# fluent/chunkio

Measured on AMD Instinct MI355X. Metric: device-resident CRC32 GB/s over N×400KB chunks; % HBM-read roofline, higher is better.
Workload: dtype u8

## Files before the change

chunkio_amd/_lib.py:

```python
import ctypes
import os
import sys

HERE = os.path.dirname(os.path.abspath(__file__))
LIB_PATH = os.environ.get("CIO_AMD_LIB") or os.path.join(HERE, "lib", "libchunkio_amd.so")

EXPORTS = (
    "crc_update",
    "cio_gpu_init", "cio_gpu_last_error", "cio_gpu_version",
    "cio_crc32_shift", "cio_crc32_combine",
    "cio_crc32_plan_create", "cio_crc32_plan_destroy", "cio_crc32_plan_exec",
    "cio_crc32_plan_exec_events", "cio_crc32_plan_bytes", "cio_crc32_plan_kernel", "cio_crc32_plan_aligned", "cio_crc32_plan_workgroups", "cio_crc32_ring_create", "cio_crc32_ring_exec",
    "cio_crc32_ring_join", "cio_crc32_ring_destroy", "cio_crc32_batch_dev", "cio_crc32_batch_host",
    "cio_crc32_devplan_create", "cio_crc32_devplan_destroy", "cio_crc32_devplan_exec", "cio_crc32_devplan_workgroups",
    "cio_crc32_batch_host_multi", "cio_crc32_split_host_multi", "cio_crc32_batch_fd_multi", "cio_gpu_device_count", "cio_gpu_set_device", "cio_gpu_get_device", "cio_gpu_numa_node",
    "cio_gpu_pci_bus_id", "cio_gpu_plan_cache_stats",
    "cio_crc32_host_register", "cio_crc32_host_unregister", "cio_gpu_pipe_last_timing",
    "cio_crc32_cpu_max", "cio_crc32_set_cpu_max", "cio_crc32_split_route", "cio_crc32_set_split_route", "cio_crc32_split_rates", "cio_crc32_split_forget", "cio_crc32_host_threads", "cio_crc32_set_host_threads",
    "cio_crc32_route_reset",
    "cio_crc32_batch_cpu", "cio_crc32_batch_fd_cpu",
    "cio_gpu_fill_synthetic", "cio_sha1_batch_dev", "cio_sha1_batch_dev_async",
    "cio_sha1_state_init", "cio_sha1_update_batch_dev", "cio_sha1_final_batch_dev", "cio_gpu_read_stream", "cio_gpu_read_stream_grid",
    "cio_gpu_event_create", "cio_gpu_event_destroy", "cio_gpu_event_record",
    "cio_gpu_event_elapsed_ms", "cio_gpu_stream_sync",
    "cio_sha1_init", "cio_sha1_update", "cio_sha1_final", "cio_sha1_hash", "cio_sha1_to_hex",
    "cioa_SHA1_Init", "cioa_SHA1_Update", "cioa_SHA1_Final",
    "cio_file_verify_batch", "cio_file_verify_batch_multi", "cio_verify_paths", "cio_verify_paths_multi",
    "cio_file_verify_batch_dev",
    "cio_dev_writer_create", "cio_dev_writer_destroy", "cio_file_init_batch_dev", "cio_file_write_batch_dev",
    "cio_file_seal_batch_dev",
    "cio_dev_writer_create_ex", "cio_dev_writer_move_segments", "cio_file_write_metadata_batch_dev",
    "cio_file_write_at_batch_dev",
    "cio_file_write_records_batch_dev",
    "cio_file_write_records_ungrouped_batch_dev",
    "cio_file_grow_batch_dev", "cio_file_grow_records_batch_dev",
    "cio_file_read_batch_dev", "cio_file_read_packed_batch_dev", "cio_meta_cmp_batch_dev",
    "cio_file_sync_batch", "cio_file_sync_batch_multi", "cio_file_sync_batch_begin", "cio_file_sync_batch_end",
    "cioa_create", "cioa_destroy", "cioa_set_max_chunks_up", "cioa_set_realloc_size_hint",
    "cioa_enable_file_trimming", "cioa_disable_file_trimming", "cioa_get_flags", "cioa_set_devices",
    "cioa_last_chunk_error", "cioa_total_chunks", "cioa_total_chunks_up",
    "cioa_stream_create", "cioa_stream_get", "cioa_stream_size_chunks_up", "cioa_stream_chunks", "cioa_scan_stream", "cioa_scan_streams", "cioa_scan_dump",
    "cioa_chunk_open", "cioa_chunk_close", "cioa_chunk_delete", "cioa_chunk_write", "cioa_chunk_write_at",
    "cioa_chunk_sync", "cioa_chunk_sync_batch", "cioa_chunk_sync_batch_begin", "cioa_chunk_sync_batch_end",
    "cioa_chunk_get_content", "cioa_chunk_get_content_copy",
    "cioa_chunk_get_content_size", "cioa_chunk_get_content_end_pos", "cioa_chunk_is_file",
    "cioa_chunk_close_stream", "cioa_chunk_get_real_size", "cioa_chunk_hash", "cioa_chunk_lock",
    "cioa_chunk_unlock", "cioa_chunk_is_locked", "cioa_chunk_tx_begin", "cioa_chunk_tx_commit",
    "cioa_chunk_tx_rollback", "cioa_chunk_is_up", "cioa_chunk_up", "cioa_chunk_up_force",
    "cioa_chunk_up_batch", "cioa_chunk_up_force_batch", "cioa_chunk_down",
    "cioa_chunk_name", "cioa_chunk_map", "cioa_error_get", "cioa_chunk_crc_cur", "cioa_chunk_set_crc_cur",
    "cioa_meta_write", "cioa_meta_read", "cioa_meta_cmp", "cioa_meta_size", "cioa_bench_perf_write",
)

_lib = None
_hip_runtime = None

c_u64_p = ctypes.POINTER(ctypes.c_uint64)
c_u32_p = ctypes.POINTER(ctypes.c_uint32)


def _bind(lib):
    V, P = ctypes.c_void_p, ctypes.POINTER
    sig = {
        "crc_update": (ctypes.c_uint64, [ctypes.c_uint64, V, ctypes.c_size_t]),
        "cio_gpu_init": (ctypes.c_int, []),
        "cio_gpu_last_error": (ctypes.c_char_p, []),
        "cio_gpu_version": (ctypes.c_char_p, []),
        "cio_crc32_shift": (ctypes.c_uint32, [ctypes.c_uint32, ctypes.c_uint64]),
        "cio_crc32_combine": (ctypes.c_uint32, [ctypes.c_uint32, ctypes.c_uint32, ctypes.c_uint64]),
        "cio_crc32_plan_create": (ctypes.c_int, [P(V), c_u64_p, c_u64_p, ctypes.c_size_t]),
        "cio_crc32_plan_destroy": (None, [V]),
        "cio_crc32_plan_exec": (ctypes.c_int, [V, V, V, V, V]),
        "cio_crc32_plan_exec_events": (ctypes.c_int, [V, V, V, V, V, V, V]),
        "cio_crc32_plan_bytes": (ctypes.c_uint64, [V]),
        "cio_crc32_plan_kernel": (ctypes.c_char_p, [V]),
        "cio_crc32_plan_workgroups": (ctypes.c_uint32, [V]),
        "cio_crc32_plan_aligned": (ctypes.c_int, [V]),
        "cio_crc32_ring_create": (ctypes.c_int, [ctypes.POINTER(V), ctypes.POINTER(ctypes.c_uint64),
                                                 ctypes.POINTER(ctypes.c_uint64), ctypes.c_size_t, ctypes.c_int]),
        "cio_crc32_ring_exec": (ctypes.c_int, [V, V, V, V, V]),
        "cio_crc32_ring_join": (ctypes.c_int, [V, V]),
        "cio_crc32_ring_destroy": (None, [V]),
        "cio_crc32_batch_dev": (ctypes.c_int, [V, c_u64_p, c_u64_p, V, V, ctypes.c_size_t, V]),
        "cio_crc32_devplan_create": (ctypes.c_int, [P(V), ctypes.c_size_t]),
        "cio_crc32_devplan_destroy": (None, [V]),
        "cio_crc32_devplan_exec": (ctypes.c_int, [V, V, ctypes.c_uint64, V, V, ctypes.c_size_t, V, V, V, V]),
        "cio_crc32_devplan_workgroups": (ctypes.c_uint32, [V]),
        "cio_file_verify_batch_dev": (ctypes.c_int, [V, V, ctypes.c_uint64, V, V, ctypes.c_size_t, ctypes.c_int,
                                                     V, V, V, V, V, V]),
        "cio_dev_writer_create": (ctypes.c_int, [P(V), ctypes.c_size_t]),
        "cio_dev_writer_destroy": (None, [V]),
        "cio_file_init_batch_dev": (ctypes.c_int, [V, V, ctypes.c_uint64, V, V, ctypes.c_size_t, V, ctypes.c_uint64,
                                                   V, V, ctypes.c_int, V, V, V]),
        "cio_file_write_batch_dev": (ctypes.c_int, [V, V, ctypes.c_uint64, V, V, ctypes.c_size_t, V, ctypes.c_uint64,
                                                    V, V, ctypes.c_int, V, V, V]),
        "cio_file_seal_batch_dev": (ctypes.c_int, [V, V, ctypes.c_uint64, V, V, ctypes.c_size_t, ctypes.c_int,
                                                   V, V, V]),
        "cio_dev_writer_create_ex": (ctypes.c_int, [P(V), ctypes.c_size_t, ctypes.c_int]),
        "cio_dev_writer_move_segments": (ctypes.c_uint32, [V]),
        "cio_file_write_metadata_batch_dev": (ctypes.c_int, [V, V, ctypes.c_uint64, V, V, ctypes.c_size_t, V,
                                                             ctypes.c_uint64, V, V, ctypes.c_int, V, V, V]),
        "cio_file_write_at_batch_dev": (ctypes.c_int, [V, V, ctypes.c_uint64, V, V, ctypes.c_size_t, V, V,
                                                       ctypes.c_uint64, V, V, ctypes.c_int, V, V, V]),
        "cio_file_write_records_batch_dev": (ctypes.c_int, [V, V, ctypes.c_uint64, V, V, ctypes.c_size_t, V,
                                                            ctypes.c_uint64, V, V, V, ctypes.c_size_t, ctypes.c_int,
                                                            V, V, V, V]),
        "cio_file_write_records_ungrouped_batch_dev": (ctypes.c_int, [V, V, ctypes.c_uint64, V, V, ctypes.c_size_t,
                                                                      V, ctypes.c_uint64, V, V, V, ctypes.c_size_t,
                                                                      ctypes.c_int, V, V, V, V, V]),
        "cio_file_grow_batch_dev": (ctypes.c_int, [V, V, ctypes.c_uint64, V, V, ctypes.c_size_t, V, V,
                                                   ctypes.c_uint64, ctypes.c_uint64, ctypes.c_uint64, ctypes.c_int,
                                                   V, V, V, V, V]),
        "cio_file_grow_records_batch_dev": (ctypes.c_int, [V, V, ctypes.c_uint64, V, V, ctypes.c_size_t, V, V,
                                                           ctypes.c_size_t, V, ctypes.c_uint64, ctypes.c_uint64,
                                                           ctypes.c_uint64, ctypes.c_int, V, V, V, V, V]),
        "cio_file_read_batch_dev": (ctypes.c_int, [V, V, ctypes.c_uint64, V, V, ctypes.c_size_t, ctypes.c_int, V,
                                                   V, ctypes.c_uint64, V, V, ctypes.c_int, V, V, V]),
        "cio_file_read_packed_batch_dev": (ctypes.c_int, [V, V, ctypes.c_uint64, V, V, ctypes.c_size_t, ctypes.c_int,
                                                          V, V, ctypes.c_uint64, ctypes.c_uint64, ctypes.c_int, V, V,
                                                          V, V, V]),
        "cio_meta_cmp_batch_dev": (ctypes.c_int, [V, ctypes.c_uint64, V, V, ctypes.c_size_t, V, ctypes.c_uint64, V,
                                                  V, V, V, V]),
        "cio_crc32_batch_host": (ctypes.c_int, [P(V), P(ctypes.c_size_t), c_u32_p, c_u32_p,
                                                ctypes.c_size_t]),
        "cio_crc32_batch_host_multi": (ctypes.c_int, [P(V), P(ctypes.c_size_t), c_u32_p, c_u32_p,
                                                      ctypes.c_size_t, P(ctypes.c_int), ctypes.c_int]),
        "cio_crc32_split_host_multi": (ctypes.c_int, [V, ctypes.c_size_t, ctypes.c_uint32, c_u32_p,
                                                      P(ctypes.c_int), ctypes.c_int]),
        "cio_gpu_device_count": (ctypes.c_int, []),
        "cio_gpu_set_device": (ctypes.c_int, [ctypes.c_int]),
        "cio_gpu_get_device": (ctypes.c_int, []),
        "cio_gpu_numa_node": (ctypes.c_int, [ctypes.c_int]),
        "cio_gpu_pci_bus_id": (ctypes.c_int, [ctypes.c_int, ctypes.c_char_p, ctypes.c_int]),
        "cio_gpu_plan_cache_stats": (ctypes.c_int, [ctypes.POINTER(ctypes.c_uint64), ctypes.c_int]),
        "cio_crc32_host_register": (ctypes.c_int, [V, ctypes.c_size_t]),
        "cio_crc32_host_unregister": (ctypes.c_int, [V]),
        "cio_gpu_pipe_last_timing": (ctypes.c_int, [P(ctypes.c_double), ctypes.c_int]),
        "cio_crc32_cpu_max": (ctypes.c_size_t, []),
        "cio_crc32_set_cpu_max": (None, [ctypes.c_size_t]),
        "cio_crc32_split_route": (ctypes.c_int, []),
        "cio_crc32_set_split_route": (None, [ctypes.c_int]),
        "cio_crc32_split_rates": (None, [ctypes.POINTER(ctypes.c_double), ctypes.c_int]),
        "cio_crc32_split_forget": (None, []),
        "cio_crc32_host_threads": (ctypes.c_int, []),
        "cio_crc32_set_host_threads": (None, [ctypes.c_int]),
        "cio_crc32_route_reset": (None, []),
        "cio_crc32_batch_cpu": (ctypes.c_int, [P(V), P(ctypes.c_size_t), c_u32_p, c_u32_p, ctypes.c_size_t,
                                               ctypes.c_int]),
        "cio_crc32_batch_fd_cpu": (ctypes.c_int, [P(ctypes.c_int), c_u64_p, P(ctypes.c_size_t), c_u32_p, c_u32_p,
                                                  ctypes.c_size_t, ctypes.c_int]),
        "cio_gpu_fill_synthetic": (ctypes.c_int, [V, c_u64_p, c_u64_p, c_u64_p, ctypes.c_size_t,
                                                  ctypes.c_uint64, V]),
        "cio_sha1_batch_dev": (ctypes.c_int, [V, c_u64_p, c_u64_p, V, ctypes.c_size_t, V]),
        "cio_sha1_batch_dev_async": (ctypes.c_int, [V, V, V, V, ctypes.c_size_t, V]),
        "cio_sha1_state_init": (None, [V, ctypes.c_size_t]),
        "cio_sha1_update_batch_dev": (ctypes.c_int, [V, V, V, V, ctypes.c_size_t, V]),
        "cio_sha1_final_batch_dev": (ctypes.c_int, [V, V, ctypes.c_size_t, V]),
        "cio_sha1_init": (None, [V]),
        "cio_sha1_update": (None, [V, V, ctypes.c_ulong]),
        "cio_sha1_final": (None, [V, V]),
# ... 98 lines not shown
```

chunkio_amd/crc32.py:

```python
import ctypes

import numpy as np

from . import _lib

CRC_INIT = 0xFFFFFFFF


def crc_init():
    return CRC_INIT


def crc_finalize(crc):
    return (crc ^ 0xFFFFFFFF) & 0xFFFFFFFF


def _as_bytes(data):
    if isinstance(data, np.ndarray):
        return np.ascontiguousarray(data).view(np.uint8)
    return np.frombuffer(memoryview(data).cast("B"), dtype=np.uint8)


def crc_update(crc, data):
    buf = _as_bytes(data)
    ptr = buf.ctypes.data if buf.size else None
    return int(_lib.lib().crc_update(crc & 0xFFFFFFFFFFFFFFFF, ptr, buf.size))


def crc32(data, seed=CRC_INIT):
    return crc_finalize(crc_update(seed, data))


def crc32_shift(raw_state, nbytes):
    return int(_lib.lib().cio_crc32_shift(raw_state & 0xFFFFFFFF, nbytes))


def crc32_combine(raw_a, raw0_b, len_b):
    return int(_lib.lib().cio_crc32_combine(raw_a & 0xFFFFFFFF, raw0_b & 0xFFFFFFFF, len_b))


def _u64_array(values):
    arr = np.ascontiguousarray(np.asarray(values, dtype=np.uint64))
    return arr, arr.ctypes.data_as(_lib.c_u64_p)


def _ptr(t):
    return None if t is None else ctypes.c_void_p(t.data_ptr())


def _stream_ptr(stream):
    if stream is None:
        import torch
        stream = torch.cuda.current_stream()
    return ctypes.c_void_p(int(stream.cuda_stream))


class Crc32Plan:

    def __init__(self, offs, lens):
        self._offs, po = _u64_array(offs)
        self._lens, pl = _u64_array(lens)
        if self._offs.shape != self._lens.shape:
            raise ValueError("offs and lens must have the same length")
        self.n = int(self._offs.size)
        handle = ctypes.c_void_p()
        _lib.check(_lib.lib().cio_crc32_plan_create(ctypes.byref(handle), po, pl, self.n),
                   "cio_crc32_plan_create")
        self._handle = handle

    @property
    def bytes(self):
        return int(_lib.lib().cio_crc32_plan_bytes(self._handle))

    @property
    def workgroups(self):
        return int(_lib.lib().cio_crc32_plan_workgroups(self._handle))

    def kernel_name(self):
        return _lib.lib().cio_crc32_plan_kernel(self._handle).decode()

    @property
    def aligned(self):
        return bool(_lib.lib().cio_crc32_plan_aligned(self._handle))

    def exec(self, base, out, seeds=None, stream=None):
        _lib.check(_lib.lib().cio_crc32_plan_exec(self._handle, _ptr(base), _ptr(seeds), _ptr(out),
                                                  _stream_ptr(stream)),
                   "cio_crc32_plan_exec")

    def exec_events(self, base, out, ev_start, ev_stop, seeds=None, stream=None):
        _lib.check(_lib.lib().cio_crc32_plan_exec_events(self._handle, _ptr(base), _ptr(seeds),
                                                         _ptr(out), _stream_ptr(stream),
                                                         ev_start, ev_stop),
                   "cio_crc32_plan_exec_events")

    def close(self):
        if getattr(self, "_handle", None):
            _lib.lib().cio_crc32_plan_destroy(self._handle)
            self._handle = None

    def __del__(self):
        try:
            self.close()
        except Exception:
            pass

    def __enter__(self):
        return self

    def __exit__(self, *exc):
        self.close()


class Crc32Ring:

    def __init__(self, offs, lens, depth=2):
        self._offs, po = _u64_array(offs)
        self._lens, pl = _u64_array(lens)
        if self._offs.shape != self._lens.shape:
            raise ValueError("offs and lens must have the same length")
        self.n = int(self._offs.size)
        handle = ctypes.c_void_p()
        _lib.check(_lib.lib().cio_crc32_ring_create(ctypes.byref(handle), po, pl, self.n, int(depth)),
                   "cio_crc32_ring_create")
        self._handle = handle

    def exec(self, base, out, seeds=None, stream=None):
        _lib.check(_lib.lib().cio_crc32_ring_exec(self._handle, _ptr(base), _ptr(seeds), _ptr(out),
                                                  _stream_ptr(stream)),
                   "cio_crc32_ring_exec")

    def join(self, stream=None):
        _lib.check(_lib.lib().cio_crc32_ring_join(self._handle, _stream_ptr(stream)), "cio_crc32_ring_join")

    def close(self):
        if getattr(self, "_handle", None):
            _lib.lib().cio_crc32_ring_destroy(self._handle)
            self._handle = None

    def __del__(self):
        try:
            self.close()
        except Exception:
            pass

    def __enter__(self):
        return self

    def __exit__(self, *exc):
        self.close()


DEVPLAN_E_BOUNDS, DEVPLAN_E_CHUNK_TOO_LARGE, DEVPLAN_E_BATCH_TOO_LARGE = 1, 2, 4


class Crc32DevPlan:

    def __init__(self, max_chunks):
        self.max_chunks = int(max_chunks)
        handle = ctypes.c_void_p()
        _lib.check(_lib.lib().cio_crc32_devplan_create(ctypes.byref(handle), self.max_chunks),
                   "cio_crc32_devplan_create")
        self._handle = handle
        import torch
        self._status = torch.zeros(1, dtype=torch.int32, device=torch.device("cuda", torch.cuda.current_device()))

# ... 304 lines not shown
```

chunkio_amd/csrc/cio_plan.h:

```cpp
#ifndef CIOA_PLAN_H
#define CIOA_PLAN_H

#include <stddef.h>
#include <stdint.h>
#include <vector>

#include "cio_diag.h"
#include "crc32_host.h"
#include "chunkio_amd/cio_crc32_gpu.h"

namespace cioa {

constexpr int kWave = 64;
constexpr int kGran = 16;
constexpr int kSub = 4;
constexpr int kRow = kWave * kGran;
constexpr int kStep = kSub * kRow;
constexpr int kThreads = 1024;
constexpr uint32_t kWavesPerWg = kThreads / kWave;
constexpr uint32_t kWfFold = 1u, kWfPublish = 2u;
constexpr int kX8Count = 2 * kStep;
constexpr uint32_t kSliceBytes = 131072;
constexpr uint32_t kShiftBytes = 32768;
constexpr uint32_t kShiftOff = kSliceBytes;
constexpr uint32_t kLdsBytes = kSliceBytes + kShiftBytes;
constexpr int kStampWords = 16;

struct ChunkDesc {
    uint64_t a;
    uint64_t vlen;
    uint64_t g;
    uint32_t nsteps;
    uint32_t h;
    uint32_t npieces;
    uint32_t w0, w1;
    uint32_t pad;
};
static_assert(sizeof(ChunkDesc) == 48, "desc layout");

struct WaveStart {
    ChunkDesc d;
    uint32_t c;
    uint32_t pad[3];
};
static_assert(sizeof(WaveStart) == 64, "wave start layout");

struct DeviceState {
    bool ready = false;
    int cus = 0;
    uint32_t *slice = nullptr;
    uint32_t *shift = nullptr;
    uint32_t *x8 = nullptr;
    uint32_t *xinv8 = nullptr;
};

struct PlanHost {
    std::vector<ChunkDesc> desc;
    std::vector<WaveStart> ws;
    std::vector<uint32_t> tiny;
    std::vector<uint32_t> pfac;
    std::vector<uint32_t> afac;
    uint64_t S = 0, bytes = 0;
};

void plan_init(cio_crc32_plan *p, DeviceState *st, size_t n);
const char *plan_build(PlanHost &ph, const uint64_t *offs, const uint64_t *lens, size_t n, uint32_t W);
const char *plan_choose(cio_crc32_plan *p, PlanHost &ph, const uint64_t *offs, const uint64_t *lens, size_t n);

constexpr int kDevHdrS = 0, kDevHdrNtiny = 1, kDevHdrBytes = 2, kDevHdrStatus = 3, kDevHdrWords = 4;
constexpr uint32_t kPlanBlock = 1024;

struct PlanBlockSum {
    uint64_t steps, bytes;
    uint32_t ntiny, err;
};

}

struct cio_crc32_plan {
    uint32_t n = 0;
    uint64_t S = 0;
    uint32_t W = 0;
    uint32_t grid = 0;
    uint32_t ntiny = 0;
    int prio = 1;
    uint64_t ustride = 0, ua0 = 0, uvlen = 0;
    uint32_t unsteps = 0, uh = 0;
    bool small = false;
    bool ahead = false;
    bool l64 = false;
    bool l64_small = false;
    bool aligned = false;
    uint32_t aq = 0, alg2p = 0;
    uint32_t *afac = nullptr;
    unsigned long long *stamps = nullptr;
    uint64_t bytes = 0;
    cioa::ChunkDesc *desc = nullptr;
    cioa::WaveStart *wstart = nullptr;
    uint32_t *tiny = nullptr;
    unsigned long long *partials = nullptr;
    uint32_t *counters = nullptr;
    uint32_t *pfac = nullptr;
    cioa::DeviceState *st = nullptr;
};

#endif
```

chunkio_amd/csrc/crc32_gpu.hip:

```cpp

#include <hip/hip_runtime.h>
#include <stdint.h>
#include <algorithm>
#include <type_traits>

#include "cio_gpu_internal.h"
#include "crc_wave.h"

using namespace cioa;

namespace {


constexpr uint32_t cx_multmodp(uint32_t a, uint32_t b)
{
    uint32_t p = 0;
    for (int i = 31; i >= 0; --i) {
        if ((a >> i) & 1u) {
            p ^= b;
        }
        b = (b & 1u) ? (b >> 1) ^ CIOA_POLY : (b >> 1);
    }
    return p;
}
// ... 1119 lines not shown
        if (L64) {
            const uint4 k1 = head_fix(make_uint4(~0u, ~0u, ~0u, ~0u), g0 + 1u, uh, 0u);
            const uint4 x1 = head_fix(make_uint4(0u, 0u, 0u, 0u), g0 + 1u, uh, 0xffffffffu);
            hk1[0] = k1.x; hk1[1] = k1.y; hk1[2] = k1.z; hk1[3] = k1.w;
            hs1[0] = x1.x; hs1[1] = x1.y; hs1[2] = x1.z; hs1[3] = x1.w;
        }
    }
    __syncthreads();

    auto chunk = [&](SmallRegs &cur, uint32_t c) {
        uint64_t a;
        uint32_t vlen, h;
        bool live;
        geom(c < c1 ? c : max(c1, 1u) - 1u, a, vlen, h, live);
        live = live && c < c1;
        uint32_t st = 0;
        const uint32_t seed = SEEDS ? cur.seed : 0xffffffffu;
        if (live) {
            StepRegs r;
#pragma unroll
            for (int q = 0; q < kSub; ++q) {
                r.q[q] = cur.q[q];
            }
            if (L64) {
                transpose64(r);
            }
            if (UNI && !SEEDS) {
                r.q[0] = make_uint4((r.q[0].x & hk[0]) ^ hs[0], (r.q[0].y & hk[1]) ^ hs[1],
                                    (r.q[0].z & hk[2]) ^ hs[2], (r.q[0].w & hk[3]) ^ hs[3]);
                if (L64) {
                    r.q[1] = make_uint4((r.q[1].x & hk1[0]) ^ hs1[0], (r.q[1].y & hk1[1]) ^ hs1[1],
                                        (r.q[1].z & hk1[2]) ^ hs1[2], (r.q[1].w & hk1[3]) ^ hs1[3]);
                }
            } else if (L64) {
                r.q[0] = head_fix(r.q[0], 4u * lane, h, seed);
                r.q[1] = head_fix(r.q[1], 4u * lane + 1u, h, seed);
            } else {
                r.q[0] = head_fix(r.q[0], lane, h, seed);
            }
            if (vlen < (uint32_t) kStep) {
#pragma unroll
                for (int q = 0; q < kSub; ++q) {
                    r.q[q] = mask_tail(r.q[q], L64 ? 64u * lane + 16u * (uint32_t) q : lbyte + (uint32_t) q * kRow,
                                       vlen);
                }
            }
            st = block16(lds, lb_lo, lb_hi, 0u, r.q[0]);
#pragma unroll
            for (int q = 1; q < kSub; ++q) {
                st = L64 ? block16(lds, lb_lo, lb_hi, st, r.q[q])
                         : shift_block16(lds, lb_lo, lb_hi, lrep, st, r.q[q]);
            }
        }
        uint32_t inv = inv_u;
        if (!UNI) {
            asm volatile("v_mov_b32 %0, %1" : "=v"(inv) : "v"(cur.inv));
        }
        issue(cur, c + 1);
        if (live) {
            uint32_t x = col[0] & (0u - (st & 1u));
#pragma unroll
            for (int j = 1; j < 32; ++j) {
                x = xor_and(x, 0u - ((st >> j) & 1u), col[j]);
            }
            uint32_t crc = wave_xor(x);
            if (vlen != (uint32_t) kStep) {
                asm volatile("" : "+v"(inv));
                crc = multmodp(inv, crc);
            }
            if (lane == 0) {
                out[c] = crc;
            }
        }
    };
    const uint32_t slot_group = __builtin_amdgcn_readfirstlane((tid >> 6) >> 2);
    for (uint32_t c = c0; c < c1; ++c) {
        rotate_prio(slot_group, c - c0);
        chunk(cur, c);
    }
    __builtin_amdgcn_s_setprio(0);
    tiny_chunks(lds, lb_lo, base, desc, tiny, seeds, out, nullptr, ntiny, wave, lane, W);
}


}

extern "C" {

int cioa_debug_stamps(const cio_crc32_plan *p, unsigned long long *host, size_t cap)
{
    if (!p || !p->stamps) {
        return 0;
    }
    const size_t n = std::min(cap, (size_t) p->W * kStampWords);
    if (hipMemcpy(host, p->stamps, n * sizeof(unsigned long long), hipMemcpyDeviceToHost) != hipSuccess) {
        return 0;
    }
    return (int) p->W;
}

int cioa_debug_plan_exec_cid(const cio_crc32_plan *p, const void *dev_base, const uint32_t *dev_seeds,
                             uint32_t *dev_out, const uint32_t *dev_cid, void *stream)
{
    return plan_exec_impl(p, dev_base, dev_seeds, dev_out, dev_cid, reinterpret_cast<hipStream_t>(stream));
}

}

using StreamKernel = decltype(&crc32_stream_kernel<false, 1, false>);

static StreamKernel select_kernel(int prio, bool stamps, bool uniform, bool ahead, bool l64)
{
    if (ahead) {
        if (l64) {
            if (stamps) {
                return crc32_stream_kernel<true, 1, true, true, true>;
            }
            return prio ? crc32_stream_kernel<false, 1, true, true, true>
                        : crc32_stream_kernel<false, 0, true, true, true>;
        }
        return prio ? crc32_stream_kernel<false, 1, true, true> : crc32_stream_kernel<false, 0, true, true>;
    }
    if (l64 && !stamps) {
        return prio ? crc32_stream_kernel<false, 1, false, false, true>
                    : crc32_stream_kernel<false, 0, false, false, true>;
    }
    switch ((prio ? 4 : 0) + (stamps ? 2 : 0) + (uniform ? 1 : 0)) {
    case 0: return crc32_stream_kernel<false, 0, false>;
    case 1: return crc32_stream_kernel<false, 0, true>;
    case 2: return crc32_stream_kernel<true, 0, false>;
    case 3: return crc32_stream_kernel<true, 0, true>;
    case 4: return crc32_stream_kernel<false, 1, false>;
    case 5: return crc32_stream_kernel<false, 1, true>;
    case 6: return crc32_stream_kernel<true, 1, false>;
    default: return crc32_stream_kernel<true, 1, true>;
    }
}


int cioa::plan_exec_impl(const cio_crc32_plan *p, const void *dev_base, const uint32_t *dev_seeds,
                         uint32_t *dev_out, const uint32_t *cid, hipStream_t s,
                         hipEvent_t ev0, hipEvent_t ev1)
{
    if (!p) {
        return fail("cio_crc32_plan_exec: null plan");
    }
    if (p->n == 0) {
        return CIO_OK;
    }
    if (!dev_base || !dev_out) {
        return fail("cio_crc32_plan_exec: null buffer");
    }
    const DeviceState *st = p->st;
    if (ev0) {
        HIP_TRY(hipEventRecord(ev0, s), "hipEventRecord");
    }
    if (p->small && !cid) {
        auto sk = p->l64_small ? (p->unsteps ? (dev_seeds ? crc32_small_kernel<true, true, true>
                                                    : crc32_small_kernel<true, false, true>)
                                       : (dev_seeds ? crc32_small_kernel<false, true, true>
                                                    : crc32_small_kernel<false, false, true>))
                         : (p->unsteps ? (dev_seeds ? crc32_small_kernel<true, true> : crc32_small_kernel<true, false>)
                                       : (dev_seeds ? crc32_small_kernel<false, true>
                                                    : crc32_small_kernel<false, false>));
        hipLaunchKernelGGL(sk, dim3(p->grid), dim3(kThreads), 0, s,
                           reinterpret_cast<const uint8_t *>(dev_base), p->ustride, p->ua0, p->uvlen, p->uh,
                           p->W, p->n, p->ntiny, st->x8, p->desc, p->tiny, dev_seeds, dev_out, st->xinv8);
        HIP_TRY(hipGetLastError(), "crc32_small_kernel launch");
        if (ev1) {
            HIP_TRY(hipEventRecord(ev1, s), "hipEventRecord");
        }
        return CIO_OK;
    }
    if (p->aligned) {
        auto ak = p->stamps ? crc32_aligned_kernel<true> : crc32_aligned_kernel<false>;
        hipLaunchKernelGGL(ak, dim3(p->grid), dim3(kThreads), 0, s, reinterpret_cast<const uint8_t *>(dev_base),
                           p->ustride, p->ua0, p->aq, p->alg2p, p->afac, dev_seeds, dev_out, cid, p->stamps);
        HIP_TRY(hipGetLastError(), "crc32_aligned_kernel launch");
        if (ev1) {
            HIP_TRY(hipEventRecord(ev1, s), "hipEventRecord");
        }
        return CIO_OK;
    }
    auto kern = select_kernel(p->prio, p->stamps != nullptr, p->unsteps != 0, p->ahead && (!p->stamps || p->l64),
                              p->l64);
    hipLaunchKernelGGL(kern, dim3(p->grid), dim3(kThreads), 0, s,
                       reinterpret_cast<const uint8_t *>(dev_base), p->S, p->ustride, p->ua0, p->uvlen,
                       p->W, p->unsteps, p->uh, p->n, p->desc, p->wstart, p->tiny,
                       dev_seeds, dev_out, cid, p->partials, p->counters, st->slice, st->shift,
                       st->x8, p->pfac, p->ntiny, p->stamps);
    HIP_TRY(hipGetLastError(), "crc32_stream_kernel launch");
    if (ev1) {
        HIP_TRY(hipEventRecord(ev1, s), "hipEventRecord");
    }
    return CIO_OK;
}

int cioa::devplan_crc_launch(const cio_crc32_plan *p, const unsigned long long *hdr, const void *dev_base,
                             const uint32_t *dev_seeds, uint32_t *dev_out, size_t n, hipStream_t s)
{
    const DeviceState *st = p->st;
    StreamKernel kern = p->l64 ? (p->prio ? crc32_stream_kernel<false, 1, false, false, true, true>
                                          : crc32_stream_kernel<false, 0, false, false, true, true>)
                               : (p->prio ? crc32_stream_kernel<false, 1, false, false, false, true>
                                          : crc32_stream_kernel<false, 0, false, false, false, true>);
    hipLaunchKernelGGL(kern, dim3(p->grid), dim3(kThreads), 0, s,
                       reinterpret_cast<const uint8_t *>(dev_base), (uint64_t) 0, (uint64_t) 0, (uint64_t) 0,
                       (uint64_t) 0, p->W, 0u, 0u, (uint32_t) n, p->desc, p->wstart, p->tiny,
                       dev_seeds, dev_out, (const uint32_t *) nullptr, p->partials, p->counters, st->slice,
                       st->shift, st->x8, p->pfac, 0u, const_cast<unsigned long long *>(hdr));
    HIP_TRY(hipGetLastError(), "crc32_stream_kernel (device-planned) launch");
    return CIO_OK;
}
```

chunkio_amd/csrc/crc_plan.cpp:

```cpp

#include <stdint.h>
#include <stdlib.h>
#include <string.h>
#include <algorithm>
#include <vector>

#include "cio_plan.h"

namespace cioa {

void plan_init(cio_crc32_plan *p, DeviceState *st, size_t n)
{
    p->st = st;
    p->n = (uint32_t) n;
    if (const char *r = cioa_diag_getenv("CIO_GPU_PRIO")) {
        const int v = atoi(r);
        p->prio = (v == 0) ? 0 : 1;
    }
    p->l64 = true;
    p->l64_small = false;
    if (const char *r = cioa_diag_getenv("CIO_GPU_L64")) {
        p->l64 = p->l64_small = atoi(r) != 0;
    }
    p->grid = (uint32_t) st->cus;
// ... 145 lines not shown
    p->ustride = stride;
    p->ua0 = ph.desc[0].a;
    p->uvlen = ph.desc[0].vlen;
    p->uh = ph.desc[0].h;
    p->unsteps = ph.desc[0].nsteps;
}

}

const char *plan_choose(cio_crc32_plan *p, PlanHost &ph, const uint64_t *offs, const uint64_t *lens, size_t n)
{
    if (const char *err = plan_build(ph, offs, lens, n, p->W)) {
        return err;
    }
    plan_uniform(p, offs, lens, n, ph);
    auto small_batch = [&ph, n] { return ph.S > 0 && ph.S == (uint64_t) n - ph.tiny.size(); };
    bool oversub = false;
    if (!cioa_diag_getenv("CIO_GPU_GRID") && ph.S >= 1024ull * p->W && 4ull * p->W <= 65536 &&
        !small_batch()) {
        PlanHost ph4;
        if (plan_build(ph4, offs, lens, n, 4 * p->W) == nullptr) {
            p->grid *= 4;
            p->W *= 4;
            oversub = true;
            ph = std::move(ph4);
        }
    }
    {
        const char *r = cioa_diag_getenv("CIO_GPU_ANTICAMP");
        const bool on = !(r && atoi(r) == 0);
        const char *mx = cioa_diag_getenv("CIO_GPU_ANTICAMP_MAX");
        const uint64_t wmax = mx ? strtoull(mx, nullptr, 10) : small_batch() ? 128 : 64;
        const uint64_t w = p->W ? ph.S / p->W : 0;
        const bool any_grid = r && atoi(r) == 2;
        if (on && (!oversub || any_grid) && !cioa_diag_getenv("CIO_GPU_GRID") && p->grid % 32 == 0 && ph.S % p->W == 0 &&
            w % 16 == 0 &&
            w > 0 && w <= wmax) {
            const uint32_t g2 = p->grid / 32 * 31;
            PlanHost ph2;
            if (plan_build(ph2, offs, lens, n, g2 * (kThreads / kWave)) == nullptr) {
                p->grid = g2;
                p->W = g2 * (kThreads / kWave);
                ph = std::move(ph2);
            }
        }
    }
    p->S = ph.S;
    p->bytes = ph.bytes;
    p->ntiny = (uint32_t) ph.tiny.size();
    p->ahead = p->unsteps != 0 && p->uh == 0 && p->uvlen % kStep == 0;
    bool short_ranges = p->S <= 64ull * p->W;
    if (const char *r = cioa_diag_getenv("CIO_GPU_AHEAD")) {
        short_ranges = atoi(r) != 0;
    }
    p->ahead = p->ahead && short_ranges;

    p->aligned = false;
    ph.afac.clear();
    {
        const char *r = cioa_diag_getenv("CIO_GPU_ALIGNED");
        const bool on = !(r && atoi(r) == 0);
        const uint64_t q = p->W ? p->S / p->W : 0;
        if (on && p->ahead && p->l64 && p->prio && p->ntiny == 0 && p->grid == (uint32_t) p->st->cus &&
            q >= 1 && q <= 64 && p->S == q * p->W && p->unsteps % q == 0) {
            const uint64_t np = p->unsteps / q;
            if (np == 2 || np == 4 || np == 8 || np == 16) {
                p->aligned = true;
                p->aq = (uint32_t) q;
                p->alg2p = np == 2 ? 1 : np == 4 ? 2 : np == 8 ? 3 : 4;
                ph.afac.resize(np * kWave);
                for (uint64_t i = 0; i < np; i++) {
                    for (uint64_t l = 0; l < (uint64_t) kWave; l++) {
                        ph.afac[i * kWave + l] = cioa_xpow8n(q * kStep * (np - 1 - i) + 64 * (kWave - 1 - l));
                    }
                }
            }
        }
    }

    p->small = small_batch();
    if (const char *r = cioa_diag_getenv("CIO_GPU_SMALL")) {
        p->small = p->small && atoi(r) != 0;
    }
    return nullptr;
}

}

using namespace cioa;

extern "C" {

int cioa_debug_plan_layout(const uint64_t *offs, const uint64_t *lens, size_t n, uint32_t W,
                           uint32_t *chunk_words, uint32_t *wave_flags)
{
    PlanHost ph;
    if (plan_build(ph, offs, lens, n, W) != nullptr) {
        return -1;
    }
    for (size_t i = 0; i < n; i++) {
        chunk_words[3 * i + 0] = ph.desc[i].w0;
        chunk_words[3 * i + 1] = ph.desc[i].w1;
        chunk_words[3 * i + 2] = ph.desc[i].npieces;
    }
    const size_t nslots = (size_t) W + n + 1;
    for (uint32_t w = 0; w < W; w++) {
        wave_flags[w] = ph.pfac[nslots + w];
    }
    return 0;
}

int cioa_debug_plan_image(const uint64_t *offs, const uint64_t *lens, size_t n, uint32_t W, void *desc,
                          void *wstart, uint32_t *tiny, uint32_t *pfac, uint64_t *hdr)
{
    PlanHost ph;
    if (plan_build(ph, offs, lens, n, W) != nullptr) {
        return -1;
    }
    memcpy(desc, ph.desc.data(), n * sizeof(ChunkDesc));
    memcpy(wstart, ph.ws.data(), (size_t) W * sizeof(WaveStart));
    if (!ph.tiny.empty()) {
        memcpy(tiny, ph.tiny.data(), ph.tiny.size() * sizeof(uint32_t));
    }
    memcpy(pfac, ph.pfac.data(), ph.pfac.size() * sizeof(uint32_t));
    hdr[kDevHdrS] = ph.S;
    hdr[kDevHdrNtiny] = ph.tiny.size();
    hdr[kDevHdrBytes] = ph.bytes;
    hdr[kDevHdrStatus] = 0;
    return 0;
}

int cioa_debug_plan_choice(const uint64_t *offs, const uint64_t *lens, size_t n, int cus, uint32_t *out_words)
{
    if (cus < 1 || n >= 0xffffffffull) {
        return -1;
    }
    DeviceState st;
    st.cus = cus;
    cio_crc32_plan p;
    PlanHost ph;
    plan_init(&p, &st, n);
    if (plan_choose(&p, ph, offs, lens, n) != nullptr) {
        return -1;
    }
    const uint64_t ntiny = p.ntiny;
    const uint32_t words[11] = {p.grid, p.W, p.small, p.ahead, p.unsteps, p.l64, p.l64_small,
                                (uint32_t) p.S, (uint32_t) (p.S >> 32), (uint32_t) ntiny, (uint32_t) (ntiny >> 32)};
    memcpy(out_words, words, sizeof(words));
    return 0;
}

int cioa_debug_plan_aligned(const uint64_t *offs, const uint64_t *lens, size_t n, int cus, uint32_t *out_words)
{
    if (cus < 1 || n >= 0xffffffffull) {
        return -1;
    }
    DeviceState st;
    st.cus = cus;
    cio_crc32_plan p;
    PlanHost ph;
    plan_init(&p, &st, n);
    if (plan_choose(&p, ph, offs, lens, n) != nullptr) {
        return -1;
    }
    out_words[0] = p.aligned;
    out_words[1] = p.aligned ? p.aq : 0;
    out_words[2] = p.aligned ? 1u << p.alg2p : 0;
    return 0;
}

}
```

chunkio_amd/csrc/gpu_runtime.hip:

```cpp

#include <hip/hip_runtime.h>
#include <stdint.h>
#include <string.h>
#include <stdio.h>
#include <stdlib.h>
#include <memory>
#include <mutex>
#include <vector>
#include <string>
#include <algorithm>

#include "cio_gpu_internal.h"

using namespace cioa;

namespace cioa {

thread_local std::string g_err;

int fail(const char *what, hipError_t e)
{
    char buf[512];
    if (e != hipSuccess) {
        snprintf(buf, sizeof(buf), "%s: %s", what, hipGetErrorString(e));
// ... 5 lines not shown
}

}

extern "C" int cioa_fail_msg(const char *what, const char *detail)
{
    g_err = std::string(what) + (detail ? std::string(": ") + detail : std::string());
    return CIO_ERROR;
}

namespace cioa {

std::mutex g_mu;
std::unique_ptr<DeviceState> g_dev[kMaxDev];

int device_state(DeviceState **out)
{
    int dev = 0;
    HIP_TRY(hipGetDevice(&dev), "hipGetDevice");
    if (dev < 0 || dev >= kMaxDev) {
        return fail("device ordinal out of range");
    }
    std::lock_guard<std::mutex> lk(g_mu);
    if (!g_dev[dev]) {
        g_dev[dev].reset(new DeviceState());
    }
    DeviceState &st = *g_dev[dev];
    if (!st.ready) {
        hipDeviceProp_t prop;
        HIP_TRY(hipGetDeviceProperties(&prop, dev), "hipGetDeviceProperties");
        if (strncmp(prop.gcnArchName, "gfx950", 6) != 0) {
            char msg[256];
            snprintf(msg, sizeof(msg), "chunkio_amd kernels are built for gfx950, device is %s",
                     prop.gcnArchName);
            return fail(msg);
        }
        st.cus = prop.multiProcessorCount;
        static uint32_t slice[4][256], shift[4][256];
        std::vector<uint32_t> x8(kX8Count);
        cioa_gen_slice4(slice);
        cioa_gen_shift_table(shift, (uint64_t) (kStep - kGran));
        cioa_gen_xpow8_table(x8.data(), kX8Count, 1);
        HIP_TRY(hipMalloc(&st.slice, sizeof(slice)), "hipMalloc(slice)");
        HIP_TRY(hipMalloc(&st.shift, sizeof(shift)), "hipMalloc(shift)");
        HIP_TRY(hipMalloc(&st.x8, kX8Count * sizeof(uint32_t)), "hipMalloc(x8)");
        HIP_TRY(hipMemcpy(st.slice, slice, sizeof(slice), hipMemcpyHostToDevice), "upload slice");
        HIP_TRY(hipMemcpy(st.shift, shift, sizeof(shift), hipMemcpyHostToDevice), "upload shift");
        HIP_TRY(hipMemcpy(st.x8, x8.data(), kX8Count * sizeof(uint32_t), hipMemcpyHostToDevice),
                "upload x8");
        std::vector<uint32_t> xinv8(kStep);
        uint32_t xm8 = 0x80000000u;
        for (int i = 0; i < 8; ++i) {
            xm8 = cioa_multmodp(xm8, (CIOA_POLY << 1) | 1u);
        }
        xinv8[0] = 0x80000000u;
        for (int d = 1; d < kStep; ++d) {
            xinv8[d] = cioa_multmodp(xinv8[d - 1], xm8);
        }
        HIP_TRY(hipMalloc(&st.xinv8, kStep * sizeof(uint32_t)), "hipMalloc(xinv8)");
        HIP_TRY(hipMemcpy(st.xinv8, xinv8.data(), kStep * sizeof(uint32_t), hipMemcpyHostToDevice),
                "upload xinv8");
        st.ready = true;
    }
    *out = &st;
    return CIO_OK;
}

}

extern "C" {

const char *cio_gpu_last_error(void)
{
    return g_err.c_str();
}

const char *cio_gpu_version(void)
{
#define CIO_STR2(x) #x
#define CIO_STR(x) CIO_STR2(x)
    return "chunkio_amd crc32 v9 gfx950 stream(l64-lanes permlane-transpose issue-ahead<=64steps wave-aligned pre-shift prio-rotate "
           "coalesced-nt division-free-start slice4-lds32x perm direct-whole preshifted-partials wg-lds-fold "
           "head-align=" CIO_STR(CIO_HEAD_ALIGN) ") "
           "small(4x16B dpp-reduce bitop3-fold prio-rotate) "
           "host(nt-staging graduated-groups pread-bounce multi-device vpclmul-crc_update small-batch-route) "
           "sha1(2-schedule-waves 4-block-handover continuation)";
}

int cio_gpu_init(void)
{
    DeviceState *st;
    return device_state(&st);
}

void cio_crc32_plan_destroy(cio_crc32_plan *p)
{
    if (!p) {
        return;
    }
    (void) hipFree(p->desc);
    (void) hipFree(p->wstart);
    (void) hipFree(p->tiny);
    (void) hipFree(p->partials);
    (void) hipFree(p->counters);
    (void) hipFree(p->pfac);
    (void) hipFree(p->afac);
    (void) hipFree(p->stamps);
    delete p;
}

int cio_crc32_plan_create(cio_crc32_plan **out, const uint64_t *offs, const uint64_t *lens, size_t n)
{
    if (!out || (n && (!offs || !lens))) {
        return fail("cio_crc32_plan_create: null argument");
    }
    if (n >= 0xffffffffull) {
        return fail("cio_crc32_plan_create: too many chunks");
    }
    *out = nullptr;
    DeviceState *st;
    if (device_state(&st) != CIO_OK) {
        return CIO_ERROR;
    }
    cio_crc32_plan *p = new cio_crc32_plan();
    plan_init(p, st, n);
    PlanHost ph;
    if (const char *err = plan_choose(p, ph, offs, lens, n)) {
        delete p;
        return fail(err);
    }
    if (const char *r = cioa_diag_getenv("CIO_GPU_STAMPS")) {
        if (atoi(r) > 0 && hipMalloc(&p->stamps, (size_t) p->W * kStampWords * sizeof(unsigned long long)) != hipSuccess) {
            p->stamps = nullptr;
        }
    }
    hipError_t e;
    const size_t npart = ph.pfac.size();
    if ((e = hipMalloc(&p->desc, ph.desc.size() * sizeof(ChunkDesc))) != hipSuccess ||
        (e = hipMalloc(&p->wstart, ph.ws.size() * sizeof(WaveStart))) != hipSuccess ||
        (e = hipMalloc(&p->tiny, std::max<size_t>(1, ph.tiny.size()) * sizeof(uint32_t))) != hipSuccess ||
        (e = hipMalloc(&p->partials, npart * sizeof(unsigned long long))) != hipSuccess ||
        (e = hipMalloc(&p->counters, std::max<size_t>(1, n) * sizeof(uint32_t))) != hipSuccess ||
        (e = hipMalloc(&p->pfac, npart * sizeof(uint32_t))) != hipSuccess ||
        (e = hipMemcpy(p->desc, ph.desc.data(), ph.desc.size() * sizeof(ChunkDesc), hipMemcpyHostToDevice)) != hipSuccess ||
        (e = hipMemcpy(p->wstart, ph.ws.data(), ph.ws.size() * sizeof(WaveStart), hipMemcpyHostToDevice)) != hipSuccess ||
        (ph.tiny.size() && (e = hipMemcpy(p->tiny, ph.tiny.data(), ph.tiny.size() * sizeof(uint32_t), hipMemcpyHostToDevice)) != hipSuccess) ||
        (e = hipMemset(p->partials, 0, npart * sizeof(unsigned long long))) != hipSuccess ||
        (e = hipMemset(p->counters, 0, std::max<size_t>(1, n) * sizeof(uint32_t))) != hipSuccess ||
        (e = hipMemcpy(p->pfac, ph.pfac.data(), npart * sizeof(uint32_t), hipMemcpyHostToDevice)) != hipSuccess ||
        (p->aligned && ((e = hipMalloc(&p->afac, ph.afac.size() * sizeof(uint32_t))) != hipSuccess ||
                        (e = hipMemcpy(p->afac, ph.afac.data(), ph.afac.size() * sizeof(uint32_t),
                                       hipMemcpyHostToDevice)) != hipSuccess))) {
        cio_crc32_plan_destroy(p);
        return fail("cio_crc32_plan_create: device allocation/upload", e);
    }
    *out = p;
    return CIO_OK;
}

uint64_t cio_crc32_plan_bytes(const cio_crc32_plan *p)
{
    return p ? p->bytes : 0;
}

uint32_t cio_crc32_plan_workgroups(const cio_crc32_plan *p)
{
    return p ? p->grid : 0;
}

const char *cio_crc32_plan_kernel(const cio_crc32_plan *p)
{
    return (p && p->small) ? "crc32_small_kernel" : "crc32_stream_kernel";
}

int cio_crc32_plan_aligned(const cio_crc32_plan *p)
{
    return (p && p->aligned) ? 1 : 0;
}

int cio_crc32_plan_exec_events(const cio_crc32_plan *p, const void *dev_base,
                               const uint32_t *dev_seeds, uint32_t *dev_out, void *stream,
                               void *ev_piece_start, void *ev_piece_stop)
{
    return plan_exec_impl(p, dev_base, dev_seeds, dev_out, nullptr,
                          reinterpret_cast<hipStream_t>(stream),
                          reinterpret_cast<hipEvent_t>(ev_piece_start),
                          reinterpret_cast<hipEvent_t>(ev_piece_stop));
}

int cio_crc32_plan_exec(const cio_crc32_plan *p, const void *dev_base, const uint32_t *dev_seeds,
                        uint32_t *dev_out, void *stream)
{
    return plan_exec_impl(p, dev_base, dev_seeds, dev_out, nullptr,
                          reinterpret_cast<hipStream_t>(stream));
}

int cio_crc32_batch_dev(const void *dev_base, const uint64_t *offs, const uint64_t *lens,
                        const uint32_t *dev_seeds, uint32_t *dev_out, size_t n, void *stream)
{
    cio_crc32_plan *p = nullptr;
    if (cio_crc32_plan_create(&p, offs, lens, n) != CIO_OK) {
        return CIO_ERROR;
    }
    int rc = cio_crc32_plan_exec(p, dev_base, dev_seeds, dev_out, stream);
    if (rc == CIO_OK) {
        hipError_t e = hipStreamSynchronize(reinterpret_cast<hipStream_t>(stream));
        if (e != hipSuccess) {
            rc = fail("cio_crc32_batch_dev: stream sync", e);
        }
    }
    cio_crc32_plan_destroy(p);
    return rc;
}

struct cio_crc32_ring {
    std::vector<cio_crc32_plan *> plans;
    std::vector<hipStream_t> streams;
    std::vector<hipEvent_t> ready, done;
    std::vector<bool> pending;
    unsigned next = 0;
    int dev = 0;
};

struct RingDevice {
    int prev = -1;
    hipError_t e = hipSuccess;
    explicit RingDevice(int dev)
    {
        if ((e = hipGetDevice(&prev)) == hipSuccess && prev != dev) {
            e = hipSetDevice(dev);
        }
    }
    ~RingDevice()
    {
        int cur = -1;
        if (prev >= 0 && hipGetDevice(&cur) == hipSuccess && cur != prev) {
            (void) hipSetDevice(prev);
        }
    }
};

void cio_crc32_ring_destroy(cio_crc32_ring *r)
{
    if (!r) {
        return;
    }
    RingDevice on(r->dev);
    for (hipStream_t st : r->streams) {
        if (st) (void) hipStreamSynchronize(st);
    }
    for (size_t i = 0; i < r->plans.size(); i++) {
        cio_crc32_plan_destroy(r->plans[i]);
        if (r->ready[i]) (void) hipEventDestroy(r->ready[i]);
        if (r->done[i]) (void) hipEventDestroy(r->done[i]);
        if (r->streams[i]) (void) hipStreamDestroy(r->streams[i]);
    }
    delete r;
}

int cio_crc32_ring_create(cio_crc32_ring **out, const uint64_t *offs, const uint64_t *lens, size_t n, int depth)
{
    if (!out) {
// ... 114 lines not shown
```

include/chunkio_amd/cio_crc32_gpu.h:

```cpp
#ifndef CIO_CRC32_GPU_H
#define CIO_CRC32_GPU_H

#include <stddef.h>
#include <stdint.h>
#include <chunkio_amd/cio_sha1_state.h>

#ifdef __cplusplus
extern "C" {
#endif

#ifndef CIO_OK
#define CIO_OK       0
#define CIO_ERROR   -1
#endif


int cio_gpu_init(void);

int cio_gpu_device_count(void);
int cio_gpu_set_device(int dev);
int cio_gpu_get_device(void);

int cio_gpu_numa_node(int dev);

int cio_gpu_pci_bus_id(int dev, char *buf, int len);

const char *cio_gpu_last_error(void);

const char *cio_gpu_version(void);


uint32_t cio_crc32_shift(uint32_t raw_state, uint64_t nbytes);

uint32_t cio_crc32_combine(uint32_t raw_a, uint32_t raw0_b, uint64_t len_b);


typedef struct cio_crc32_plan cio_crc32_plan;

int  cio_crc32_plan_create(cio_crc32_plan **plan, const uint64_t *offs,
                           const uint64_t *lens, size_t n);
void cio_crc32_plan_destroy(cio_crc32_plan *plan);

int  cio_crc32_plan_exec(const cio_crc32_plan *plan, const void *dev_base,
                         const uint32_t *dev_seeds, uint32_t *dev_out,
                         void *stream);

int  cio_crc32_plan_exec_events(const cio_crc32_plan *plan, const void *dev_base,
                                const uint32_t *dev_seeds, uint32_t *dev_out,
                                void *stream, void *ev_piece_start,
                                void *ev_piece_stop);

uint64_t cio_crc32_plan_bytes(const cio_crc32_plan *plan);

const char *cio_crc32_plan_kernel(const cio_crc32_plan *plan);

int cio_crc32_plan_aligned(const cio_crc32_plan *plan);

typedef struct cio_crc32_ring cio_crc32_ring;
int  cio_crc32_ring_create(cio_crc32_ring **ring, const uint64_t *offs, const uint64_t *lens, size_t n, int depth);
int  cio_crc32_ring_exec(cio_crc32_ring *ring, const void *dev_base, const uint32_t *dev_seeds, uint32_t *dev_out,
                         void *stream);
int  cio_crc32_ring_join(cio_crc32_ring *ring, void *stream);
void cio_crc32_ring_destroy(cio_crc32_ring *ring);

uint32_t cio_crc32_plan_workgroups(const cio_crc32_plan *plan);

int  cio_crc32_batch_dev(const void *dev_base, const uint64_t *offs,
                         const uint64_t *lens, const uint32_t *dev_seeds,
                         uint32_t *dev_out, size_t n, void *stream);

typedef struct cio_crc32_devplan cio_crc32_devplan;

#define CIO_DEVPLAN_E_BOUNDS           1
#define CIO_DEVPLAN_E_CHUNK_TOO_LARGE  2
#define CIO_DEVPLAN_E_BATCH_TOO_LARGE  4

int  cio_crc32_devplan_create(cio_crc32_devplan **plan, size_t max_chunks);
void cio_crc32_devplan_destroy(cio_crc32_devplan *plan);

int  cio_crc32_devplan_exec(cio_crc32_devplan *plan, const void *dev_base, uint64_t dev_bytes,
                            const uint64_t *dev_offs, const uint64_t *dev_lens, size_t n,
                            const uint32_t *dev_seeds, uint32_t *dev_out,
                            uint32_t *dev_status, void *stream);

uint32_t cio_crc32_devplan_workgroups(const cio_crc32_devplan *plan);


int  cio_crc32_batch_host(const void *const *bufs, const size_t *lens,
                          const uint32_t *seeds, uint32_t *out_raw, size_t n);

int  cio_crc32_batch_host_multi(const void *const *bufs, const size_t *lens,
                                const uint32_t *seeds, uint32_t *out_raw, size_t n,
                                const int *devices, int ndev);

int  cio_crc32_split_host_multi(const void *buf, size_t len, uint32_t seed, uint32_t *out_raw,
                                const int *devices, int ndev);

int  cio_crc32_batch_fd_multi(const int *fds, const uint64_t *foffs, const size_t *lens,
                              const uint32_t *seeds, uint32_t *out_raw, size_t n,
                              const int *devices, int ndev);

int  cio_crc32_host_register(const void *p, size_t len);
int  cio_crc32_host_unregister(const void *p);

int  cio_gpu_pipe_last_timing(double *out, int n);

int  cio_gpu_plan_cache_stats(uint64_t *out, int n);


int  cio_crc32_batch_cpu(const void *const *bufs, const size_t *lens,
                         const uint32_t *seeds, uint32_t *out_raw, size_t n,
                         int threads);
int  cio_crc32_batch_fd_cpu(const int *fds, const uint64_t *foffs, const size_t *lens,
                            const uint32_t *seeds, uint32_t *out_raw, size_t n,
                            int threads);

size_t cio_crc32_cpu_max(void);
void   cio_crc32_set_cpu_max(size_t bytes);
int    cio_crc32_split_route(void);
void   cio_crc32_set_split_route(int on);
void   cio_crc32_split_rates(double *out, int n);
void   cio_crc32_split_forget(void);
int    cio_crc32_host_threads(void);
void   cio_crc32_set_host_threads(int threads);
void   cio_crc32_route_reset(void);


int  cio_gpu_fill_synthetic(void *dev_base, const uint64_t *offs,
                            const uint64_t *lens, const uint64_t *ids, size_t n,
                            uint64_t seed, void *stream);


int  cio_sha1_batch_dev(const void *dev_base, const uint64_t *offs,
                        const uint64_t *lens, uint8_t *dev_digests, size_t n,
                        void *stream);

int  cio_sha1_batch_dev_async(const void *dev_base, const uint64_t *dev_offs,
                              const uint64_t *dev_lens, uint8_t *dev_digests,
                              size_t n, void *stream);
// ... 30 lines not shown
```

Measured before the change: 6558.

## Add small-aligned CRC32 kernel with double-buffered loads for uniform-stride chunk batches

```diff
diff --git a/chunkio_amd/_lib.py b/chunkio_amd/_lib.py
--- a/chunkio_amd/_lib.py
+++ b/chunkio_amd/_lib.py
@@ -10,7 +10,7 @@
     "cio_gpu_init", "cio_gpu_last_error", "cio_gpu_version",
     "cio_crc32_shift", "cio_crc32_combine",
     "cio_crc32_plan_create", "cio_crc32_plan_destroy", "cio_crc32_plan_exec",
-    "cio_crc32_plan_exec_events", "cio_crc32_plan_bytes", "cio_crc32_plan_kernel", "cio_crc32_plan_aligned", "cio_crc32_plan_workgroups", "cio_crc32_ring_create", "cio_crc32_ring_exec",
+    "cio_crc32_plan_exec_events", "cio_crc32_plan_bytes", "cio_crc32_plan_kernel", "cio_crc32_plan_aligned", "cio_crc32_plan_small_aligned", "cio_crc32_plan_workgroups", "cio_crc32_ring_create", "cio_crc32_ring_exec",
     "cio_crc32_ring_join", "cio_crc32_ring_destroy", "cio_crc32_batch_dev", "cio_crc32_batch_host",
     "cio_crc32_devplan_create", "cio_crc32_devplan_destroy", "cio_crc32_devplan_exec", "cio_crc32_devplan_workgroups",
     "cio_crc32_batch_host_multi", "cio_crc32_split_host_multi", "cio_crc32_batch_fd_multi", "cio_gpu_device_count", "cio_gpu_set_device", "cio_gpu_get_device", "cio_gpu_numa_node",
@@ -76,6 +76,7 @@
         "cio_crc32_plan_kernel": (ctypes.c_char_p, [V]),
         "cio_crc32_plan_workgroups": (ctypes.c_uint32, [V]),
         "cio_crc32_plan_aligned": (ctypes.c_int, [V]),
+        "cio_crc32_plan_small_aligned": (ctypes.c_int, [V]),
         "cio_crc32_ring_create": (ctypes.c_int, [ctypes.POINTER(V), ctypes.POINTER(ctypes.c_uint64),
                                                  ctypes.POINTER(ctypes.c_uint64), ctypes.c_size_t, ctypes.c_int]),
         "cio_crc32_ring_exec": (ctypes.c_int, [V, V, V, V, V]),
diff --git a/chunkio_amd/crc32.py b/chunkio_amd/crc32.py
--- a/chunkio_amd/crc32.py
+++ b/chunkio_amd/crc32.py
@@ -82,6 +82,10 @@
     @property
     def aligned(self):
         return bool(_lib.lib().cio_crc32_plan_aligned(self._handle))
+
+    @property
+    def small_aligned(self):
+        return bool(_lib.lib().cio_crc32_plan_small_aligned(self._handle))
 
     def exec(self, base, out, seeds=None, stream=None):
         _lib.check(_lib.lib().cio_crc32_plan_exec(self._handle, _ptr(base), _ptr(seeds), _ptr(out),
diff --git a/chunkio_amd/csrc/cio_plan.h b/chunkio_amd/csrc/cio_plan.h
--- a/chunkio_amd/csrc/cio_plan.h
+++ b/chunkio_amd/csrc/cio_plan.h
@@ -93,6 +93,8 @@
     bool aligned = false;
     uint32_t aq = 0, alg2p = 0;
     uint32_t *afac = nullptr;
+    bool small_aligned = false;
+    uint32_t sak = 0;
     unsigned long long *stamps = nullptr;
     uint64_t bytes = 0;
     cioa::ChunkDesc *desc = nullptr;
diff --git a/chunkio_amd/csrc/crc32_gpu.hip b/chunkio_amd/csrc/crc32_gpu.hip
--- a/chunkio_amd/csrc/crc32_gpu.hip
+++ b/chunkio_amd/csrc/crc32_gpu.hip
@@ -1225,6 +1225,119 @@
     tiny_chunks(lds, lb_lo, base, desc, tiny, seeds, out, nullptr, ntiny, wave, lane, W);
 }
 
+template <bool SEEDS>
+__global__ void __launch_bounds__(kThreads, 1)
+crc32_small_aligned_kernel(const uint8_t *base, uint64_t ustride, uint64_t ua0, uint32_t k,
+                           const uint32_t *__restrict__ g_x8, const uint32_t *__restrict__ seeds, uint32_t *out)
+{
+    __shared__ __attribute__((aligned(16))) char lds[kLdsBytes];
+    const uint32_t tid = threadIdx.x;
+    const uint32_t wslot = __builtin_amdgcn_readfirstlane(tid >> 6);
+    const uint32_t wave = blockIdx.x * (uint32_t) kWavesPerWg + wslot;
+    const uint32_t lane = tid & 63u;
+    const uint32_t c0 = wave * k;
+    const uint32_t loff = 64u * (lane & 15u) + 16u * (lane >> 4);
+    const uint8_t *cnext = base + (ua0 + (uint64_t) c0 * ustride);
+    auto load = [&](StepRegs &r, uint32_t &seed, uint32_t c) {
+#pragma unroll
+        for (int q = 0; q < kSub; ++q) {
+            r.q[q] = ldg16(cnext + loff + (uint32_t) q * kRow);
+        }
+        if (SEEDS) {
+            seed = load_vec_u32(seeds + c);
+        }
+        cnext += ustride;
+    };
+
+    StepRegs cur, nxt;
+    uint32_t seed_cur = 0xffffffffu, seed_nxt = 0xffffffffu;
+    load(cur, seed_cur, c0);
+    __builtin_amdgcn_sched_barrier(0);
+    const uint32_t xl = g_x8[64u * (63u - lane)];
+    __builtin_amdgcn_sched_barrier(0);
+    const uint32_t lb_lo = (lane & kSliceRepMask) << 2;
+    const uint32_t lb_hi = lb_lo | 0x10000u;
+    const uint32_t slot_group = wslot >> 2;
+    {
+        uint32_t tab_v[kE], tab_sv[kE];
+        table_entries<cx_xpow8n(kRow - kGran)>(__builtin_amdgcn_readfirstlane(tid >> 8), tid & 255u, tab_v[0],
+                                               tab_sv[0]);
+        write_tables(lds, tid, tab_v, tab_sv);
+    }
+    __syncthreads();
+
+    auto landed = [](StepRegs &r, uint32_t &seed) {
+        asm volatile("" : "+v"(r.q[0].x), "+v"(r.q[0].y), "+v"(r.q[0].z), "+v"(r.q[0].w),
+                          "+v"(r.q[1].x), "+v"(r.q[1].y), "+v"(r.q[1].z), "+v"(r.q[1].w),
+                          "+v"(r.q[2].x), "+v"(r.q[2].y), "+v"(r.q[2].z), "+v"(r.q[2].w),
+                          "+v"(r.q[3].x), "+v"(r.q[3].y), "+v"(r.q[3].z), "+v"(r.q[3].w));
+        if (SEEDS) {
+            asm volatile("" : "+v"(seed));
+        }
+    };
+    uint32_t col[32];
+    uint32_t res = 0;
+    auto half = [&](uint32_t it, StepRegs &use, uint32_t &seed_use, StepRegs &fill, uint32_t &seed_fill,
+                    auto refill, auto first) {
+        rotate_prio(slot_group, it);
+        landed(use, seed_use);
+        if (decltype(refill)::value) {
+            load(fill, seed_fill, c0 + it + 1u);
+            __builtin_amdgcn_sched_barrier(0);
+        }
+        if (decltype(first)::value) {
+            col[31] = xl;
+#pragma unroll
+            for (int j = 30; j >= 0; --j) {
+                col[j] = (col[j + 1] >> 1) ^ (CIOA_POLY & (0u - (col[j + 1] & 1u)));
+            }
+#pragma unroll
+            for (int j = 0; j < 32; j += 8) {
+                asm volatile("" : "+v"(col[j]), "+v"(col[j + 1]), "+v"(col[j + 2]), "+v"(col[j + 3]),
+                                  "+v"(col[j + 4]), "+v"(col[j + 5]), "+v"(col[j + 6]), "+v"(col[j + 7]));
+            }
+        }
+        transpose64(use);
+        use.q[0].x ^= lane == 0 ? seed_use : 0u;
+        uint32_t st = block16(lds, lb_lo, lb_hi, 0u, use.q[0]);
+#pragma unroll
+        for (int q = 1; q < kSub; ++q) {
+            st = block16(lds, lb_lo, lb_hi, st, use.q[q]);
+        }
+        uint32_t acc[4] = {0u, 0u, 0u, 0u};
+#pragma unroll
+        for (int j = 0; j < 32; ++j) {
+            acc[j & 3] = xor_and(acc[j & 3], 0u - ((st >> j) & 1u), col[j]);
+        }
+        const uint32_t crc = wave_xor(xor3(acc[0], acc[1], acc[2]) ^ acc[3]);
+        res = lane == it ? crc : res;
+    };
+    using Refill = std::true_type;
+    using NoRefill = std::false_type;
+    using First = std::true_type;
+    using Later = std::false_type;
+    if (k == 1) {
+        half(0, cur, seed_cur, nxt, seed_nxt, NoRefill(), First());
+    } else {
+        half(0, cur, seed_cur, nxt, seed_nxt, Refill(), First());
+        uint32_t it = 1;
+        for (; it + 2 < k; it += 2) {
+            half(it, nxt, seed_nxt, cur, seed_cur, Refill(), Later());
+            half(it + 1, cur, seed_cur, nxt, seed_nxt, Refill(), Later());
+        }
+        if (k - it == 2) {
+            half(it, nxt, seed_nxt, cur, seed_cur, Refill(), Later());
+            half(it + 1, cur, seed_cur, nxt, seed_nxt, NoRefill(), Later());
+        } else {
+            half(it, nxt, seed_nxt, cur, seed_cur, NoRefill(), Later());
+        }
+    }
+    __builtin_amdgcn_s_setprio(0);
+    if (lane < k) {
+        out[c0 + lane] = res;
+    }
+}
+
 
 }
 
@@ -1297,6 +1410,16 @@
     const DeviceState *st = p->st;
     if (ev0) {
         HIP_TRY(hipEventRecord(ev0, s), "hipEventRecord");
+    }
+    if (p->small_aligned && !cid) {
+        auto ak = dev_seeds ? crc32_small_aligned_kernel<true> : crc32_small_aligned_kernel<false>;
+        hipLaunchKernelGGL(ak, dim3(p->grid), dim3(kThreads), 0, s, reinterpret_cast<const uint8_t *>(dev_base),
+                           p->ustride, p->ua0, p->sak, st->x8, dev_seeds, dev_out);
+        HIP_TRY(hipGetLastError(), "crc32_small_aligned_kernel launch");
+        if (ev1) {
+            HIP_TRY(hipEventRecord(ev1, s), "hipEventRecord");
+        }
+        return CIO_OK;
     }
     if (p->small && !cid) {
         auto sk = p->l64_small ? (p->unsteps ? (dev_seeds ? crc32_small_kernel<true, true, true>
diff --git a/chunkio_amd/csrc/crc_plan.cpp b/chunkio_amd/csrc/crc_plan.cpp
--- a/chunkio_amd/csrc/crc_plan.cpp
+++ b/chunkio_amd/csrc/crc_plan.cpp
@@ -251,6 +251,20 @@
     if (const char *r = cioa_diag_getenv("CIO_GPU_SMALL")) {
         p->small = p->small && atoi(r) != 0;
     }
+
+    p->small_aligned = false;
+    p->sak = 0;
+    {
+        const char *r = cioa_diag_getenv("CIO_GPU_SMALL_ALIGNED");
+        const bool on = !(r && atoi(r) == 0);
+        const uint64_t k = p->W ? (uint64_t) n / p->W : 0;
+        if (on && p->small && p->unsteps != 0 && p->uvlen == (uint64_t) kStep && p->uh == 0 && p->ntiny == 0 &&
+            p->prio && !cioa_diag_getenv("CIO_GPU_GRID") && p->grid == (uint32_t) p->st->cus && k >= 1 && k <= 64 &&
+            (uint64_t) n == k * p->W) {
+            p->small_aligned = true;
+            p->sak = (uint32_t) k;
+        }
+    }
     return nullptr;
 }
 
@@ -338,4 +352,22 @@
     return 0;
 }
 
-}
+int cioa_debug_plan_small_aligned(const uint64_t *offs, const uint64_t *lens, size_t n, int cus, uint32_t *out_words)
+{
+    if (cus < 1 || n >= 0xffffffffull) {
+        return -1;
+    }
+    DeviceState st;
+    st.cus = cus;
+    cio_crc32_plan p;
+    PlanHost ph;
+    plan_init(&p, &st, n);
+    if (plan_choose(&p, ph, offs, lens, n) != nullptr) {
+        return -1;
+    }
+    out_words[0] = p.small_aligned;
+    out_words[1] = p.small_aligned ? p.sak : 0;
+    return 0;
+}
+
+}
diff --git a/chunkio_amd/csrc/gpu_runtime.hip b/chunkio_amd/csrc/gpu_runtime.hip
--- a/chunkio_amd/csrc/gpu_runtime.hip
+++ b/chunkio_amd/csrc/gpu_runtime.hip
@@ -111,7 +111,7 @@
     return "chunkio_amd crc32 v9 gfx950 stream(l64-lanes permlane-transpose issue-ahead<=64steps wave-aligned pre-shift prio-rotate "
            "coalesced-nt division-free-start slice4-lds32x perm direct-whole preshifted-partials wg-lds-fold "
            "head-align=" CIO_STR(CIO_HEAD_ALIGN) ") "
-           "small(4x16B dpp-reduce bitop3-fold prio-rotate) "
+           "small(4x16B dpp-reduce bitop3-fold prio-rotate small-aligned-l64-issue-ahead) "
            "host(nt-staging graduated-groups pread-bounce multi-device vpclmul-crc_update small-batch-route) "
            "sha1(2-schedule-waves 4-block-handover continuation)";
 }
@@ -207,6 +207,11 @@
     return (p && p->aligned) ? 1 : 0;
 }
 
+int cio_crc32_plan_small_aligned(const cio_crc32_plan *p)
+{
+    return (p && p->small_aligned) ? 1 : 0;
+}
+
 int cio_crc32_plan_exec_events(const cio_crc32_plan *p, const void *dev_base,
                                const uint32_t *dev_seeds, uint32_t *dev_out, void *stream,
                                void *ev_piece_start, void *ev_piece_stop)
diff --git a/include/chunkio_amd/cio_crc32_gpu.h b/include/chunkio_amd/cio_crc32_gpu.h
--- a/include/chunkio_amd/cio_crc32_gpu.h
+++ b/include/chunkio_amd/cio_crc32_gpu.h
@@ -55,6 +55,8 @@
 const char *cio_crc32_plan_kernel(const cio_crc32_plan *plan);
 
 int cio_crc32_plan_aligned(const cio_crc32_plan *plan);
+
+int cio_crc32_plan_small_aligned(const cio_crc32_plan *plan);
 
 typedef struct cio_crc32_ring cio_crc32_ring;
 int  cio_crc32_ring_create(cio_crc32_ring **ring, const uint64_t *offs, const uint64_t *lens, size_t n, int depth);
```

New measurement: 6427. -2.0%, worse.
